# JiehongLin/SAM-6D

Measured on NVIDIA H100. Metric: poses/sec, higher is better.
Workload: dtype bf16

## Files before the change

include/sam6d_b200.h:

```cpp
#ifndef SAM6D_B200_H
#define SAM6D_B200_H

#ifdef __cplusplus
extern "C" {
#endif


int sam6d_fps(const float* xyz, int b, int n, int m, float* temp, int* idx, void* stream);
int sam6d_fps_single_cta(const float* xyz, int b, int n, int m, float* temp, int* idx, void* stream);

int sam6d_gather_points(const float* points, const int* idx, int b, int c, int n, int m, float* out, void* stream);

int sam6d_gather_rows(const float* src, const int* idx, int b, int n, int m, int c, long long src_bstride, float* out,
                      void* stream);
int sam6d_gather_rows_bf16_f32(const void* src, const int* idx, int b, int n, int m, int c, long long src_bstride, float* out,
                               void* stream);

int sam6d_ball_query(const float* new_xyz, const float* xyz, int b, int n, int m, float radius, int nsample, int* idx,
                     int* cnt, void* stream);
int sam6d_ball_query_pair(const float* new_xyz, const float* xyz, int b, int n, int m, float radius_a, int nsample_a,
                          float radius_b, int nsample_b, int* idx_a, int* idx_b, int* cnt_a, int* cnt_b, void* stream);

int sam6d_group_points(const float* points, const int* idx, int b, int c, int n, int np, int ns, float* out, void* stream);

// ... 123 lines not shown
int sam6d_attn_tc_ex(const void* Q, long long q_ld, int q_col0, const void* K, long long k_ld, int k_col0, const void* Vt,
                     long long vt_ld, int B, int H, int Sq, int Sk, int head_dim, float scale, int k_brows, int k_row0, int v_col0,
                     float* lse, void* out, int out_is_bf16, long long out_ld, void* stream);
int sam6d_attn_merge_key(const void* Q, long long q_ld, int q_col0, const void* K, long long k_ld, int k_col0, int k_brows,
                         int key_row, const void* Vt, long long vt_ld, int key_col, const float* lse, int B, int H, int Sq,
                         float scale, void* out, long long out_ld, void* stream);
int sam6d_transpose_tokens_bf16(const void* src, long long ld, int col0, int C, int nB, int L, int N1, void* out, void* stream);
int sam6d_linattn_kv(const float* Kf, long long k_ld, long long k_bs, const float* V, long long v_ld, long long v_bs, int B,
                     int H, int J, float* KV, float* KS, void* stream);
int sam6d_linattn_apply(const float* Qf, long long q_rpb, long long q_bs, long long q_ld, const float* KV, const float* KS,
                        int B, int H, float* X, long long x_bs, long long x_ld, void* stream);
int sam6d_linattn_kv_pack(const float* Kf, long long k_ld, long long k_bs, const float* V, long long v_ld, long long v_bs, int B,
                          int J, void* blob, float* KS, void* stream);
int sam6d_linattn_tc(const void* Q, long long q_ld, long long q_bs, const void* blob, const float* KS,
                     const float* softplus_scale, int B, int rpb, void* X, long long x_ld, long long x_bs, void* stream);

int sam6d_coarse_assign(const float* A, int B, int S, float* W, float* w1, void* stream);
int sam6d_coarse_sample(const float* W, int B, int L, const float* rand, int nr, int* idx, void* stream);
int sam6d_coarse_hypotheses(const int* idx, const float* pts1, const float* pts2, int B, int n, int n1, float* Rt,
                            float* resid, void* stream);
int sam6d_topk_smallest(const float* v, int B, int n, int k, int* out, void* stream);
int sam6d_coarse_select(const float* Rt, const int* top, int B, int n1, int n2, const float* pts1, const float* w1, int n,
                        const float* model, int nm, float* scores, float* R, float* t, void* stream);
int sam6d_coarse_pick_distinct(const float* Rt, const int* top, const float* scores, int B, int n1, int n2, int K, float cos_thr,
                               float d2_min, float* R_out, float* t_out, float* score_out, unsigned char* valid, int* count,
                               void* stream);
int sam6d_coarse_pick_distinct_sym(const float* Rt, const int* top, const float* scores, int B, int n1, int n2, int K, float cos_thr,
                                   float d2_min, const float* symR, const float* symt, int S, const int* sym_range, int max_count,
                                   const float* radius, float* R_out, float* t_out, float* score_out, unsigned char* valid,
                                   int* count, void* stream);
// ... 95 lines not shown
```

sam6d_b200/csrc/linattn_tc.cu:

```cuda
#include "tc.cuh"

namespace {

constexpr int H = 4, D = 64, C = H * D;
constexpr int A_SLAB = 128 * 128;
constexpr int B_SLAB = 64 * 128;
constexpr int BLOB_BYTES = H * B_SLAB;
constexpr int LT_THREADS = 256;
constexpr int LT_SMEM = H * A_SLAB + H * B_SLAB + 128 * H * 4 + 1024;

__global__ void __launch_bounds__(1024) linattn_kv_pack_kernel(const float* __restrict__ Kf, long long k_ld, long long k_bs,
                                                               const float* __restrict__ V, long long v_ld, long long v_bs, int J,
                                                               uint8_t* __restrict__ blob, float* __restrict__ KS) {
  extern __shared__ __align__(16) float sm[];
  float* ks = sm;
  float* vs = ks + J * D;
  const int bh = blockIdx.x, b = bh / H, h = bh - b * H, tid = threadIdx.x;
  for (int e = tid; e < J * D; e += 1024) {
    int j = e / D, c = e - j * D;
    ks[e] = Kf[(size_t)b * k_bs + (size_t)j * k_ld + h * D + c];
    vs[e] = V[(size_t)b * v_bs + (size_t)j * v_ld + h * D + c];
  }
  __syncthreads();
  const int d = tid >> 4, e0 = (tid & 15) * 4;
  float4 acc = make_float4(0.f, 0.f, 0.f, 0.f);
  float ksum = 0.f;
#pragma unroll 4
  for (int j = 0; j < J; ++j) {
    const float kd = ks[j * D + d];
    const float4 v = *reinterpret_cast<const float4*>(vs + j * D + e0);
    ksum += kd;
    acc.x = fmaf(kd, v.x, acc.x); acc.y = fmaf(kd, v.y, acc.y); acc.z = fmaf(kd, v.z, acc.z); acc.w = fmaf(kd, v.w, acc.w);
  }
  uint8_t* slab = blob + (size_t)b * BLOB_BYTES + h * B_SLAB;
  *reinterpret_cast<__nv_bfloat16*>(slab + tc::sw128_offset(e0 + 0, d)) = __float2bfloat16(acc.x);
  *reinterpret_cast<__nv_bfloat16*>(slab + tc::sw128_offset(e0 + 1, d)) = __float2bfloat16(acc.y);
// ... 15 lines not shown
  uint8_t* a_s = smem;
  uint8_t* b_s = smem + H * A_SLAB;
  float* zs = reinterpret_cast<float*>(b_s + H * B_SLAB);
  __shared__ __align__(8) uint64_t blob_bar;

  const int tid = threadIdx.x, warp = tid >> 5, lane = tid & 31;
  const int b = blockIdx.x / a.tiles_per_cloud, tile = blockIdx.x - b * a.tiles_per_cloud;
  if (tid == 0) {
    tc::mbar_init(&blob_bar, 1);
    tc::mbar_fence_init();
    tc::mbar_arrive_expect_tx(&blob_bar, BLOB_BYTES);
    tc::bulk_load_1d(b_s, a.blob + (size_t)b * BLOB_BYTES, BLOB_BYTES, &blob_bar);
  }

  float rs[8], ksv[8];
  {
    const float4 s0 = *reinterpret_cast<const float4*>(a.sp_scale + lane * 8), s1 = *reinterpret_cast<const float4*>(a.sp_scale + lane * 8 + 4);
    rs[0] = 1.f / s0.x; rs[1] = 1.f / s0.y; rs[2] = 1.f / s0.z; rs[3] = 1.f / s0.w;
    rs[4] = 1.f / s1.x; rs[5] = 1.f / s1.y; rs[6] = 1.f / s1.z; rs[7] = 1.f / s1.w;
    const float4 k0 = *reinterpret_cast<const float4*>(a.KS + (size_t)b * C + lane * 8), k1 = *reinterpret_cast<const float4*>(a.KS + (size_t)b * C + lane * 8 + 4);
    ksv[0] = k0.x; ksv[1] = k0.y; ksv[2] = k0.z; ksv[3] = k0.w; ksv[4] = k1.x; ksv[5] = k1.y; ksv[6] = k1.z; ksv[7] = k1.w;
  }
  const int head = lane >> 3, piece = lane & 7;
  const __nv_bfloat16* qbase = a.Q + (size_t)b * a.q_bs + (size_t)tile * 128 * a.q_ld + lane * 8;
  const int rows_left = a.rpb - tile * 128;
#pragma unroll 1
  for (int i0 = warp; i0 < 128; i0 += 32) {
    uint4 raw[4];
#pragma unroll
    for (int u = 0; u < 4; ++u) {
      const int i = i0 + u * 8;
      raw[u] = (i < rows_left) ? *reinterpret_cast<const uint4*>(qbase + (size_t)i * a.q_ld) : make_uint4(0u, 0u, 0u, 0u);
    }
#pragma unroll
    for (int u = 0; u < 4; ++u) {
      const int i = i0 + u * 8;
      const uint32_t w[4] = {raw[u].x, raw[u].y, raw[u].z, raw[u].w};
      float q[8];
      float s1 = 0.f, s3 = 0.f;
#pragma unroll
      for (int e = 0; e < 4; ++e) {
        q[2 * e] = __uint_as_float(w[e] << 16);
        q[2 * e + 1] = __uint_as_float(w[e] & 0xffff0000u);
      }
#pragma unroll
      for (int e = 0; e < 8; ++e) {
        float t = (fmaxf(q[e], 0.f) + 1e-6f) * rs[e];
        s1 = fmaf(t, t, s1);
        t = t * t * t;
        s3 = fmaf(t, t, s3);
        q[e] = t;
      }
      s1 = warp_sum(s1);
      s3 = warp_sum(s3);
      const float n = sqrtf(s1) * rsqrtf(s3);
      float zp = 0.f;
#pragma unroll
      for (int e = 0; e < 8; ++e) { q[e] *= n; zp = fmaf(q[e], ksv[e], zp); }
      zp += __shfl_xor_sync(0xffffffffu, zp, 1);
      zp += __shfl_xor_sync(0xffffffffu, zp, 2);
      zp += __shfl_xor_sync(0xffffffffu, zp, 4);
      const bool valid = i < rows_left;
      if (piece == 0) zs[i * H + head] = valid ? 1.f / (zp + 1e-6f) : 0.f;
      uint4 o = make_uint4(0u, 0u, 0u, 0u);
      if (valid) o = make_uint4(tc::pack_bf16(q[0], q[1]), tc::pack_bf16(q[2], q[3]), tc::pack_bf16(q[4], q[5]), tc::pack_bf16(q[6], q[7]));
      *reinterpret_cast<uint4*>(a_s + head * A_SLAB + i * 128 + ((piece ^ (i & 7)) << 4)) = o;
    }
  }
  tc::fence_proxy_async_smem();
  __syncthreads();

  const int wg = warp >> 2, w = warp & 3;
  tc::mbar_wait(&blob_bar, 0);
  __nv_bfloat16* xb = a.X + (size_t)b * a.x_bs;
#pragma unroll 1
  for (int h = 0; h < H; ++h) {
    float acc[D / 2];
    const uint32_t a_addr = tc::smem_u32(a_s + h * A_SLAB) + wg * (64 * 128), b_addr = tc::smem_u32(b_s + h * B_SLAB);
    tc::wg_fence();
#pragma unroll
// ... 1 lines not shown
    tc::wg_commit();
    tc::wg_wait<0>();
#pragma unroll
    for (int hr = 0; hr < 2; ++hr) {
      const int r = wg * 64 + tc::frag_row(2 * hr, w, lane), row = tile * 128 + r;
      if (row >= a.rpb) continue;
      const float z = zs[r * H + h];
#pragma unroll
      for (int j = 0; j < D / 8; ++j)
        *reinterpret_cast<uint32_t*>(xb + (size_t)row * a.x_ld + h * D + tc::frag_col(4 * j, lane)) =
            tc::pack_bf16(acc[4 * j + 2 * hr] * z, acc[4 * j + 2 * hr + 1] * z);
    }
  }
}

}

S6_API int sam6d_linattn_kv_pack(const float* Kf, long long k_ld, long long k_bs, const float* V, long long v_ld, long long v_bs,
                                 int B, int J, void* blob, float* KS, void* stream) {
  S6_REQUIRE(Kf && V && blob && KS && B >= 0 && J > 0);
  if (B == 0) return 0;
  size_t smem = (size_t)2 * J * D * sizeof(float);
  S6_REQUIRE(smem <= 200 * 1024);
  S6_CHECK(cudaFuncSetAttribute(linattn_kv_pack_kernel, cudaFuncAttributeMaxDynamicSharedMemorySize, (int)smem));
  linattn_kv_pack_kernel<<<B * H, 1024, smem, s6_stream(stream)>>>(Kf, k_ld, k_bs, V, v_ld, v_bs, J, reinterpret_cast<uint8_t*>(blob), KS);
  S6_LAUNCH_CHECK();
  return 0;
}

S6_API int sam6d_linattn_tc(const void* Q, long long q_ld, long long q_bs, const void* blob, const float* KS,
                            const float* softplus_scale, int B, int rpb, void* X, long long x_ld, long long x_bs, void* stream) {
  S6_REQUIRE(Q && blob && KS && softplus_scale && X && B >= 0 && rpb >= 0 && (q_ld % 8) == 0 && (x_ld % 8) == 0 &&
             (q_bs % 8) == 0 && (x_bs % 8) == 0);
  S6_REQUIRE((reinterpret_cast<uintptr_t>(Q) & 15) == 0 && (reinterpret_cast<uintptr_t>(X) & 15) == 0 &&
             (reinterpret_cast<uintptr_t>(blob) & 15) == 0 && (long long)B * rpb < 2000000000LL);
  if (B == 0 || rpb == 0) return 0;
  S6_CHECK(cudaFuncSetAttribute(linattn_tc_kernel, cudaFuncAttributeMaxDynamicSharedMemorySize, LT_SMEM));
  LtArgs a{reinterpret_cast<const __nv_bfloat16*>(Q), q_ld, q_bs, reinterpret_cast<const uint8_t*>(blob), KS, softplus_scale,
           reinterpret_cast<__nv_bfloat16*>(X), x_ld, x_bs, rpb, s6_cdiv(rpb, 128)};
  linattn_tc_kernel<<<B * a.tiles_per_cloud, LT_THREADS, LT_SMEM, s6_stream(stream)>>>(a);
  S6_LAUNCH_CHECK();
  return 0;
// ... 2 lines not shown
```

sam6d_b200/csrc/rowops.cu:

```cuda
#include "common.cuh"

namespace {

struct RowView {
  long long rpb, bstride, ld;
  __device__ __forceinline__ size_t off(long long r) const {
    long long b = r / rpb, i = r - b * rpb;
    return (size_t)(b * bstride + i * ld);
  }
};

constexpr int MAXV_LIMIT = 64;

__device__ __forceinline__ void st_out(float* p, float v) { *p = v; }
__device__ __forceinline__ void st_out(__nv_bfloat16* p, float v) { *p = __float2bfloat16(v); }

__device__ __forceinline__ float ld_in(const float* p) { return *p; }
__device__ __forceinline__ float ld_in(const __nv_bfloat16* p) { return __bfloat162float(*p); }

template <int MAXV, typename OT, typename IT = float>
__global__ void __launch_bounds__(256) layernorm_kernel(const IT* __restrict__ x, RowView xv, OT* __restrict__ y, RowView yv,
                                                        const float* __restrict__ gamma, const float* __restrict__ beta,
                                                        long long rows, int C, float eps) {
  const int lane = threadIdx.x & 31;
// ... 113 lines not shown
  const float n = fmaxf(sqrtf(warp_sum(s)), 1e-12f);
#pragma unroll
  for (int i = 0; i < MAXV; ++i)
    if (i < nv) st_out(yp + lane + 32 * i, v[i] / n);
}

template <int MAXV>
__global__ void __launch_bounds__(256) focus_kernel(const float* __restrict__ x, RowView xv, float* __restrict__ y, RowView yv,
                                                    const float* __restrict__ sp_scale, long long rows, int C) {
  const int lane = threadIdx.x & 31;
  const long long r = (long long)blockIdx.x * 8 + (threadIdx.x >> 5);
  if (r >= rows) return;
  const float* xp = x + xv.off(r);
  float* yp = y + yv.off(r);
  const int nv = C >> 5;
  float v[MAXV];
  float s1 = 0.f, s3 = 0.f;
#pragma unroll
  for (int i = 0; i < MAXV; ++i)
    if (i < nv) {
      int c = lane + 32 * i;
      float q = (fmaxf(xp[c], 0.f) + 1e-6f) / sp_scale[c];
      s1 += q * q;
      q = q * q * q;
      s3 += q * q;
      v[i] = q;
    }
  const float n1 = sqrtf(warp_sum(s1)), n3 = sqrtf(warp_sum(s3));
#pragma unroll
  for (int i = 0; i < MAXV; ++i)
    if (i < nv) yp[lane + 32 * i] = (v[i] / n3) * n1;
}

__global__ void rigid_warp_kernel(const float* __restrict__ p, const float* __restrict__ R, const float* __restrict__ t, int n,
                                  long long total, float* __restrict__ out) {
  long long i = (long long)blockIdx.x * blockDim.x + threadIdx.x;
  if (i >= total) return;
  int b = (int)(i / n);
  const float* Rb = R + (size_t)b * 9;
  const float* tb = t + (size_t)b * 3;
  float x = p[i * 3 + 0] - tb[0], y = p[i * 3 + 1] - tb[1], z = p[i * 3 + 2] - tb[2];
  out[i * 3 + 0] = x * Rb[0] + y * Rb[3] + z * Rb[6];
  out[i * 3 + 1] = x * Rb[1] + y * Rb[4] + z * Rb[7];
// ... 165 lines not shown
```

sam6d_b200/csrc/tail_tc.cu:

```cuda
#include "tc.cuh"

namespace {

constexpr int BM = 128, C = 256, HID = 512, BK = 64;
constexpr int T_SLAB = BM * 128;
constexpr int T_BYTES = 4 * T_SLAB;
constexpr int W_STAGE = 256 * 128;
constexpr int W_STAGES = 3;
constexpr int W_PER_TILE = 20;
constexpr int CONSUMERS = 256, THREADS = CONSUMERS + 128;
constexpr int SMEM = 2 * T_BYTES + W_STAGES * W_STAGE + 1024;

struct TailArgs {
  const float* bo; const float* g1; const float* b1;
  const float* be; const float* bs; const float* g2; const float* b2;
  int M;
  float eps;
};

__device__ __forceinline__ uint32_t* tile_pair(uint8_t* tile, int r, int col) {
  return reinterpret_cast<uint32_t*>(tile + (col >> 6) * T_SLAB + r * 128 + ((((col & 63) >> 3) ^ (r & 7)) << 4) + (col & 7) * 2);
}
__device__ __forceinline__ float2 unpack2(uint32_t w) { return make_float2(__uint_as_float(w << 16), __uint_as_float(w & 0xffff0000u)); }

__global__ void __launch_bounds__(THREADS, 1) tail_tc_kernel(const __grid_constant__ CUtensorMap tmHid, const __grid_constant__ CUtensorMap tmX,
                                                const __grid_constant__ CUtensorMap tmWo, const __grid_constant__ CUtensorMap tmWe,
                                                const __grid_constant__ CUtensorMap tmWs, TailArgs a, __nv_bfloat16* __restrict__ out,
                                                long long ld_out) {
  extern __shared__ __align__(1024) uint8_t smem_raw[];
  uint8_t* smem = reinterpret_cast<uint8_t*>((reinterpret_cast<uintptr_t>(smem_raw) + 1023) & ~(uintptr_t)1023);
  uint8_t* a_buf = smem;
  uint8_t* x_buf = smem + T_BYTES;
  uint8_t* w_ring = smem + 2 * T_BYTES;
  __shared__ __align__(8) uint64_t in_full, in_empty, w_full[W_STAGES], w_empty[W_STAGES];

  const int tid = threadIdx.x, warp = tid >> 5, lane = tid & 31;
  const int ntiles = (a.M + BM - 1) / BM;

  if (tid == 0) {
    tc::mbar_init(&in_full, 1); tc::mbar_init(&in_empty, CONSUMERS / 32);
    for (int s = 0; s < W_STAGES; ++s) { tc::mbar_init(&w_full[s], 1); tc::mbar_init(&w_empty[s], CONSUMERS / 32); }
    tc::mbar_fence_init();
    tc::tma_prefetch_desc(&tmHid); tc::tma_prefetch_desc(&tmX); tc::tma_prefetch_desc(&tmWo);
    tc::tma_prefetch_desc(&tmWe); tc::tma_prefetch_desc(&tmWs);
  }
  s6_pdl_trigger();
  if (tid < CONSUMERS) {
    for (int i = tid; i < 512; i += CONSUMERS) {
      const float* p = i < 64 ? a.bo + i * 4 : i < 128 ? a.g1 + (i - 64) * 4 : i < 192 ? a.b1 + (i - 128) * 4 : i < 320 ? a.be + (i - 192) * 4
                     : i < 384 ? a.bs + (i - 320) * 4 : i < 448 ? a.g2 + (i - 384) * 4 : a.b2 + (i - 448) * 4;
      asm volatile("prefetch.global.L1 [%0];" ::"l"(p));
    }
  }
  __syncthreads();
  s6_pdl_wait();

  if (warp >= CONSUMERS / 32) {
    tc::producer_regs();
    if (tid == CONSUMERS) {
      long long gw = 0;
      int it = 0;
      for (int tile = blockIdx.x; tile < ntiles; tile += gridDim.x, ++it) {
        const int m0 = tile * BM;
        auto load_w = [&](int j) {
          const int s = (int)(gw % W_STAGES);
          tc::mbar_wait(&w_empty[s], (uint32_t)(((gw / W_STAGES) & 1) ^ 1));
          tc::mbar_arrive_expect_tx(&w_full[s], W_STAGE);
          uint8_t* dst = w_ring + s * W_STAGE;
          if (j < 4) tc::tma_load_2d(&tmWo, &w_full[s], dst, j * BK, 0);
          else if (j < 12) tc::tma_load_2d(&tmWe, &w_full[s], dst, ((j - 4) & 3) * BK, ((j - 4) >> 2) * 256);
          else tc::tma_load_2d(&tmWs, &w_full[s], dst, (j - 12) * BK, 0);
          ++gw;
        };
        int j = 0;
        for (; j < W_STAGES; ++j) load_w(j);
        tc::mbar_wait(&in_empty, (uint32_t)((it & 1) ^ 1));
        tc::mbar_arrive_expect_tx(&in_full, 2 * T_BYTES);
#pragma unroll
        for (int kb = 0; kb < 4; ++kb) {
          tc::tma_load_2d(&tmHid, &in_full, a_buf + kb * T_SLAB, kb * BK, m0);
          tc::tma_load_2d(&tmX, &in_full, x_buf + kb * T_SLAB, kb * BK, m0);
        }
        for (; j < W_PER_TILE; ++j) load_w(j);
      }
    }
    return;
  }
  tc::consumer_regs();
  const int wg = warp >> 2, w = warp & 3;
  const uint32_t a_addr = tc::smem_u32(a_buf) + wg * (64 * 128), x_addr = tc::smem_u32(x_buf) + wg * (64 * 128), w_addr0 = tc::smem_u32(w_ring);
  long long gw = 0;
  float acc[C / 2];
  auto gemm = [&](uint32_t op_addr, uint32_t op_addr2, int nkb) {
    int prev = -1;
    for (int kb = 0; kb < nkb; ++kb, ++gw) {
      const int s = (int)(gw % W_STAGES);
      tc::mbar_wait(&w_full[s], (uint32_t)((gw / W_STAGES) & 1));
      const uint32_t op = (kb < 4 ? op_addr : op_addr2) + (kb & 3) * T_SLAB;
      tc::wg_fence();
#pragma unroll
      for (int k = 0; k < 4; ++k)
        tc::wgmma_bf16<C>(acc, tc::wg_desc(op + k * 32), tc::wg_desc(w_addr0 + s * W_STAGE + k * 32), (kb | k) ? 1u : 0u);
      tc::wg_commit();
      if (prev >= 0) {
// ... 31 lines not shown
  };
  auto relu_store = [&](const float* __restrict__ bias, uint8_t* dst) {
#pragma unroll
    for (int e = 0; e < C / 2; e += 2) {
      const int col = tc::frag_col(e, lane), r = wg * 64 + tc::frag_row(e, w, lane);
      const float2 bb = __ldg(reinterpret_cast<const float2*>(bias + col));
      *tile_pair(dst, r, col) = tc::pack_bf16(fmaxf(acc[e] + bb.x, 0.f), fmaxf(acc[e + 1] + bb.y, 0.f));
    }
  };
  auto publish = [&]() {
    tc::fence_proxy_async_smem();
    tc::named_bar(1 + wg, 128);
  };
  int it = 0;
  for (int tile = blockIdx.x; tile < ntiles; tile += gridDim.x, ++it) {
    tc::mbar_wait(&in_full, (uint32_t)(it & 1));
    gemm(a_addr, a_addr, 4);
    layernorm(a.bo, a.g1, a.b1, [&](int e, int hr, int col) {
      return unpack2(*tile_pair(x_buf, wg * 64 + tc::frag_row(e, w, lane), col));
    });
#pragma unroll
    for (int e = 0; e < C / 2; e += 2) {
      const int r = wg * 64 + tc::frag_row(e, w, lane), col = tc::frag_col(e, lane), row = tile * BM + r;
      const uint32_t y2 = tc::pack_bf16(acc[e], acc[e + 1]);
      *tile_pair(a_buf, r, col) = y2;
      if (row < a.M) *reinterpret_cast<uint32_t*>(out + (size_t)row * ld_out + col) = y2;
    }
    publish();
    gemm(a_addr, a_addr, 4);
    relu_store(a.be, x_buf);
    gemm(a_addr, a_addr, 4);
    tc::named_bar(1 + wg, 128);
    relu_store(a.be + 256, a_buf);
    publish();
    gemm(x_addr, a_addr, 8);
    if (lane == 0) tc::mbar_arrive(&in_empty);
    layernorm(a.bs, a.g2, a.b2, [&](int e, int, int col) {
      const int row = tile * BM + wg * 64 + tc::frag_row(e, w, lane);
      return row < a.M ? unpack2(*reinterpret_cast<const uint32_t*>(out + (size_t)row * ld_out + col)) : make_float2(0.f, 0.f);
    });
#pragma unroll
    for (int e = 0; e < C / 2; e += 2) {
      const int row = tile * BM + wg * 64 + tc::frag_row(e, w, lane);
      if (row < a.M) *reinterpret_cast<uint32_t*>(out + (size_t)row * ld_out + tc::frag_col(e, lane)) = tc::pack_bf16(acc[e], acc[e + 1]);
    }
  }
}

}

S6_API int sam6d_transformer_tail_bf16(const void* hid, long long ld_hid, const void* x, long long ld_x, const void* Wo, const float* bo,
                                       const float* g1, const float* b1, const void* We, const float* be, const void* Ws, const float* bs,
                                       const float* g2, const float* b2, void* out, long long ld_out, int M, float eps, void* stream) {
  S6_REQUIRE(hid && x && Wo && bo && g1 && b1 && We && be && Ws && bs && g2 && b2 && out && M >= 0);
  S6_REQUIRE((ld_hid % 8) == 0 && (ld_x % 8) == 0 && (ld_out % 8) == 0 && ld_hid >= C && ld_x >= C && ld_out >= C);
  S6_REQUIRE(((reinterpret_cast<uintptr_t>(hid) | reinterpret_cast<uintptr_t>(x) | reinterpret_cast<uintptr_t>(out) | reinterpret_cast<uintptr_t>(Wo) |
               reinterpret_cast<uintptr_t>(We) | reinterpret_cast<uintptr_t>(Ws) | reinterpret_cast<uintptr_t>(bo) | reinterpret_cast<uintptr_t>(be) |
               reinterpret_cast<uintptr_t>(bs) | reinterpret_cast<uintptr_t>(g1) | reinterpret_cast<uintptr_t>(b1) | reinterpret_cast<uintptr_t>(g2) |
               reinterpret_cast<uintptr_t>(b2)) & 15) == 0);
  if (M == 0) return 0;
  CUtensorMap tmHid, tmX, tmWo, tmWe, tmWs;
  int rc;
  if ((rc = tc::make_map_2d(&tmHid, hid, M, C, ld_hid, 64, BM))) return rc;
  if ((rc = tc::make_map_2d(&tmX, x, M, C, ld_x, 64, BM))) return rc;
  if ((rc = tc::make_map_2d(&tmWo, Wo, C, C, C, 64, 256))) return rc;
  if ((rc = tc::make_map_2d(&tmWe, We, HID, C, C, 64, 256))) return rc;
  if ((rc = tc::make_map_2d(&tmWs, Ws, C, HID, HID, 64, 256))) return rc;
  int grid;
  S6_CHECK(s6_persistent_grid(s6_cdiv(M, BM), 1, &grid));
  TailArgs a{bo, g1, b1, be, bs, g2, b2, M, eps};
  S6_CHECK(cudaFuncSetAttribute(tail_tc_kernel, cudaFuncAttributeMaxDynamicSharedMemorySize, SMEM));
  S6_CHECK(s6_launch_pdl(tail_tc_kernel, dim3(grid), dim3(THREADS), SMEM, s6_stream(stream), tmHid, tmX, tmWo, tmWe, tmWs, a,
                         reinterpret_cast<__nv_bfloat16*>(out), ld_out));
  S6_LAUNCH_CHECK();
  return 0;
}
```

sam6d_b200/ops.py:

```python
from typing import Optional, Tuple

import numpy as np
import torch

from . import _lib

Tensor = torch.Tensor


def _check(t: Tensor, dtype, name: str, ndim: Optional[int] = None):
    if not isinstance(t, torch.Tensor):
        raise RuntimeError(f"{name} must be a torch.Tensor")
    if not t.is_cuda:
        raise RuntimeError(f"{name} must be a CUDA tensor (CPU not supported)")
    if t.dtype != dtype:
        raise RuntimeError(f"{name} must be {dtype}, got {t.dtype}")
    if not t.is_contiguous():
        raise RuntimeError(f"{name} must be contiguous")
    if ndim is not None and t.dim() != ndim:
        raise RuntimeError(f"{name} must have {ndim} dims, got {t.dim()}")


def _rows(t: Tensor) -> Tuple[int, int, int]:
    if t.dim() not in (2, 3) or t.stride(-1) != 1:
# ... 524 lines not shown


def linattn_apply(q: Tensor, KV: Tensor, KS: Tensor, out: Tensor):
    _, x_bs, x_ld = _rows(out)
    _lib.call("sam6d_linattn_apply", q, *_rows(q), KV, KS, q.shape[0], KV.shape[1], out, x_bs, x_ld)


def linattn_kv_pack(k: Tensor, v: Tensor) -> Tuple[Tensor, Tensor]:
    B, J, _ = k.shape
    _, k_bs, k_ld = _rows(k)
    _, v_bs, v_ld = _rows(v)
    blob = torch.empty(B, 4 * 64 * 64, dtype=torch.bfloat16, device=k.device)
    KS = torch.empty(B, 4, 64, dtype=torch.float32, device=k.device)
    _lib.call("sam6d_linattn_kv_pack", k, k_ld, k_bs, v, v_ld, v_bs, B, J, blob, KS)
    return blob, KS


def linattn_tc(q: Tensor, blob: Tensor, KS: Tensor, sp_scale: Tensor, out: Tensor):
    B, rpb, _ = q.shape
    _, q_bs, q_ld = _rows(q)
    _, x_bs, x_ld = _rows(out)
    _lib.call("sam6d_linattn_tc", q, q_ld, q_bs, blob, KS, sp_scale, B, rpb, out, x_ld, x_bs)


def coarse_assign(A: Tensor) -> Tuple[Tensor, Tensor]:
    _check(A, torch.float32, "atten", 3)
    B, S, _ = A.shape
    n = S - 1
    W = torch.empty(B, n * n, dtype=torch.float32, device=A.device)
    w1 = torch.empty(B, n, dtype=torch.float32, device=A.device)
# ... 471 lines not shown
```

sam6d_b200/pem.py:

```python
import math
from types import SimpleNamespace
from typing import Dict, Optional

import torch
import torch.nn as nn

from . import ops
from .layers import _W, _f32, _gemm, _Packed, _param_key, PRECISIONS

NUM_HEADS = 4

RPE_TC = True
PADDED_BIAS = True
GEO_LUT_INV_H = 8.0
GEO_LUT_D_MAX = 32.0


def _cfg(cfg, **defaults):
    if isinstance(cfg, dict):
        cfg = SimpleNamespace(**cfg)
    for k, v in defaults.items():
        if not hasattr(cfg, k):
            setattr(cfg, k, v)
    return cfg
# ... 488 lines not shown
    def _pack(self):
        la = self.dense_layer.attention.attention
        return dict(
            wq=_W(la.proj_q.weight), bq=_f32(la.proj_q.bias),
            wkv=_W(torch.cat([_f32(la.proj_k.weight), _f32(la.proj_v.weight)], dim=0)),
            bkv=torch.cat([_f32(la.proj_k.bias), _f32(la.proj_v.bias)], dim=0).contiguous(),
            sp_scale=torch.nn.functional.softplus(_f32(la.scale)).reshape(-1).contiguous(), tail=_pack_tail(self.dense_layer))

    def _sample_feats(self, dense_feats, idx_ext):
        if dense_feats.dtype == torch.bfloat16:
            return ops.gather_rows_bf16(dense_feats, idx_ext)
        return ops.gather_rows(dense_feats, idx_ext)

    def _dense_layer_bf16(self, dense, sparse, w):
        B, N1, C = dense.shape
        N, J = N1 - 1, sparse.shape[1] - 1
        dev = dense.device
        bf = torch.bfloat16
        x2d = dense.view(B * N1, C)
        q = ops.gemm_tma(x2d, w["wq"].bf16, w["bq"], out_dtype=bf)
        kv = torch.empty(B * J, 2 * C, dtype=torch.float32, device=dev)
        ops.gemm_tc(sparse[:, 1:, :], w["wkv"].bf16, w["bkv"], out=kv.view(B, J, 2 * C))
        ops.focus_rows(kv[:, :C], w["sp_scale"], out=kv[:, :C])
        kv3 = kv.view(B, J, 2 * C)
        blob, KS = ops.linattn_kv_pack(kv3[..., :C], kv3[..., C:])
        x_att = torch.empty(B * N1, C, dtype=bf, device=dev)
        ops.linattn_tc(q.view(B, N1, C)[:, 1:, :], blob, KS, w["sp_scale"], x_att.view(B, N1, C)[:, 1:, :])
        x_att.view(B, N1, C)[:, 0, :] = 0
        out = _tail_bf16(x2d, x_att, w["tail"]).view(B, N1, C)
        out[:, 0, :] = sparse[:, 0, :].to(bf)
        return out

    def _dense_layer(self, dense, sparse, w):
        B, N1, C = dense.shape
        N, J = N1 - 1, sparse.shape[1] - 1
        dev = dense.device
        x = dense[:, 1:, :]
        q = torch.empty(B * N, C, dtype=torch.float32, device=dev)
        prec = self.precision
        _gemm(prec, x, w["wq"], w["bq"], out=q.view(B, N, C))
        kv = torch.empty(B * J, 2 * C, dtype=torch.float32, device=dev)
        _gemm(prec, sparse[:, 1:, :], w["wkv"], w["bkv"], out=kv.view(B, J, 2 * C))
        ops.focus_rows(q, w["sp_scale"], out=q)
        ops.focus_rows(kv[:, :C], w["sp_scale"], out=kv[:, :C])
        KV = torch.empty(B, NUM_HEADS, 64, 64, dtype=torch.float32, device=dev)
        KS = torch.empty(B, NUM_HEADS, 64, dtype=torch.float32, device=dev)
# ... 269 lines not shown
```

Measured before the change: 2635.

## Fuse Q projection and linear attention into the persistent tail kernel

```diff
diff --git a/include/sam6d_b200.h b/include/sam6d_b200.h
--- a/include/sam6d_b200.h
+++ b/include/sam6d_b200.h
@@ -161,6 +161,12 @@
                           int J, void* blob, float* KS, void* stream);
 int sam6d_linattn_tc(const void* Q, long long q_ld, long long q_bs, const void* blob, const float* KS,
                      const float* softplus_scale, int B, int rpb, void* X, long long x_ld, long long x_bs, void* stream);
+int sam6d_linattn_kv_focus_pack(const float* K, long long k_ld, long long k_bs, const float* V, long long v_ld, long long v_bs,
+                                const float* softplus_scale, int B, int J, void* blob, float* KS, void* stream);
+int sam6d_linattn_tail_bf16(const void* x, long long ld_x, int B, int N1, const void* Wq, const float* bq, const void* blob,
+                            const float* KS, const float* softplus_scale, const void* bg, long long bg_bs, const void* Wo,
+                            const float* bo, const float* g1, const float* b1, const void* We, const float* be, const void* Ws,
+                            const float* bs, const float* g2, const float* b2, void* out, long long ld_out, float eps, void* stream);
 
 int sam6d_coarse_assign(const float* A, int B, int S, float* W, float* w1, void* stream);
 int sam6d_coarse_sample(const float* W, int B, int L, const float* rand, int nr, int* idx, void* stream);
diff --git a/sam6d_b200/csrc/linattn.cuh b/sam6d_b200/csrc/linattn.cuh
--- /dev/null
+++ b/sam6d_b200/csrc/linattn.cuh
@@ -0,0 +1,64 @@
+#pragma once
+#include "tc.cuh"
+
+namespace linattn {
+
+template <int MAXV>
+__device__ __forceinline__ void focus_f32_row(const float* __restrict__ xp, const float* __restrict__ sp_scale, int nv, int lane,
+                                              float (&v)[MAXV], float& n1, float& n3) {
+  float s1 = 0.f, s3 = 0.f;
+#pragma unroll
+  for (int i = 0; i < MAXV; ++i)
+    if (i < nv) {
+      int c = lane + 32 * i;
+      float q = (fmaxf(xp[c], 0.f) + 1e-6f) / sp_scale[c];
+      s1 += q * q;
+      q = q * q * q;
+      s3 += q * q;
+      v[i] = q;
+    }
+  n1 = sqrtf(warp_sum(s1));
+  n3 = sqrtf(warp_sum(s3));
+}
+
+__device__ __forceinline__ uint4 focus_bf16_row(uint4 raw, const float (&rs)[8], const float (&ksv)[8], bool valid, float& zinv) {
+  const uint32_t w[4] = {raw.x, raw.y, raw.z, raw.w};
+  float q[8];
+  float s1 = 0.f, s3 = 0.f;
+#pragma unroll
+  for (int e = 0; e < 4; ++e) {
+    q[2 * e] = __uint_as_float(w[e] << 16);
+    q[2 * e + 1] = __uint_as_float(w[e] & 0xffff0000u);
+  }
+#pragma unroll
+  for (int e = 0; e < 8; ++e) {
+    float t = (fmaxf(q[e], 0.f) + 1e-6f) * rs[e];
+    s1 = fmaf(t, t, s1);
+    t = t * t * t;
+    s3 = fmaf(t, t, s3);
+    q[e] = t;
+  }
+  s1 = warp_sum(s1);
+  s3 = warp_sum(s3);
+  const float n = sqrtf(s1) * rsqrtf(s3);
+  float zp = 0.f;
+#pragma unroll
+  for (int e = 0; e < 8; ++e) { q[e] *= n; zp = fmaf(q[e], ksv[e], zp); }
+  zp += __shfl_xor_sync(0xffffffffu, zp, 1);
+  zp += __shfl_xor_sync(0xffffffffu, zp, 2);
+  zp += __shfl_xor_sync(0xffffffffu, zp, 4);
+  zinv = valid ? 1.f / (zp + 1e-6f) : 0.f;
+  if (!valid) return make_uint4(0u, 0u, 0u, 0u);
+  return make_uint4(tc::pack_bf16(q[0], q[1]), tc::pack_bf16(q[2], q[3]), tc::pack_bf16(q[4], q[5]), tc::pack_bf16(q[6], q[7]));
+}
+
+__device__ __forceinline__ void focus_bf16_consts(const float* __restrict__ sp_scale, const float* __restrict__ KS, int b, int lane,
+                                                  float (&rs)[8], float (&ksv)[8]) {
+  const float4 s0 = *reinterpret_cast<const float4*>(sp_scale + lane * 8), s1 = *reinterpret_cast<const float4*>(sp_scale + lane * 8 + 4);
+  rs[0] = 1.f / s0.x; rs[1] = 1.f / s0.y; rs[2] = 1.f / s0.z; rs[3] = 1.f / s0.w;
+  rs[4] = 1.f / s1.x; rs[5] = 1.f / s1.y; rs[6] = 1.f / s1.z; rs[7] = 1.f / s1.w;
+  const float4 k0 = *reinterpret_cast<const float4*>(KS + (size_t)b * 256 + lane * 8), k1 = *reinterpret_cast<const float4*>(KS + (size_t)b * 256 + lane * 8 + 4);
+  ksv[0] = k0.x; ksv[1] = k0.y; ksv[2] = k0.z; ksv[3] = k0.w; ksv[4] = k1.x; ksv[5] = k1.y; ksv[6] = k1.z; ksv[7] = k1.w;
+}
+
+}
diff --git a/sam6d_b200/csrc/linattn_tc.cu b/sam6d_b200/csrc/linattn_tc.cu
--- a/sam6d_b200/csrc/linattn_tc.cu
+++ b/sam6d_b200/csrc/linattn_tc.cu
@@ -1,4 +1,4 @@
-#include "tc.cuh"
+#include "linattn.cuh"
 
 namespace {
 
@@ -9,17 +9,37 @@
 constexpr int LT_THREADS = 256;
 constexpr int LT_SMEM = H * A_SLAB + H * B_SLAB + 128 * H * 4 + 1024;
 
-__global__ void __launch_bounds__(1024) linattn_kv_pack_kernel(const float* __restrict__ Kf, long long k_ld, long long k_bs,
+template <bool FOCUS>
+__global__ void __launch_bounds__(1024, 1) linattn_kv_pack_kernel(const float* __restrict__ Kf, long long k_ld, long long k_bs,
                                                                const float* __restrict__ V, long long v_ld, long long v_bs, int J,
-                                                               uint8_t* __restrict__ blob, float* __restrict__ KS) {
+                                                               const float* __restrict__ sp_scale, uint8_t* __restrict__ blob,
+                                                               float* __restrict__ KS) {
   extern __shared__ __align__(16) float sm[];
   float* ks = sm;
   float* vs = ks + J * D;
   const int bh = blockIdx.x, b = bh / H, h = bh - b * H, tid = threadIdx.x;
-  for (int e = tid; e < J * D; e += 1024) {
-    int j = e / D, c = e - j * D;
-    ks[e] = Kf[(size_t)b * k_bs + (size_t)j * k_ld + h * D + c];
-    vs[e] = V[(size_t)b * v_bs + (size_t)j * v_ld + h * D + c];
+  if constexpr (FOCUS) {
+    const int warp = tid >> 5, lane = tid & 31;
+    for (int j = warp; j < J; j += 32) {
+      float v[8], n1, n3;
+      linattn::focus_f32_row(Kf + (size_t)b * k_bs + (size_t)j * k_ld, sp_scale, 8, lane, v, n1, n3);
+      float lo = v[0], hi = v[1];
+#pragma unroll
+      for (int i = 2; i < 8; i += 2)
+        if ((i >> 1) == h) { lo = v[i]; hi = v[i + 1]; }
+      ks[j * D + lane] = (lo / n3) * n1;
+      ks[j * D + lane + 32] = (hi / n3) * n1;
+    }
+    for (int e = tid; e < J * D; e += 1024) {
+      int j = e / D, c = e - j * D;
+      vs[e] = V[(size_t)b * v_bs + (size_t)j * v_ld + h * D + c];
+    }
+  } else {
+    for (int e = tid; e < J * D; e += 1024) {
+      int j = e / D, c = e - j * D;
+      ks[e] = Kf[(size_t)b * k_bs + (size_t)j * k_ld + h * D + c];
+      vs[e] = V[(size_t)b * v_bs + (size_t)j * v_ld + h * D + c];
+    }
   }
   __syncthreads();
   const int d = tid >> 4, e0 = (tid & 15) * 4;
@@ -65,13 +85,7 @@
   }
 
   float rs[8], ksv[8];
-  {
-    const float4 s0 = *reinterpret_cast<const float4*>(a.sp_scale + lane * 8), s1 = *reinterpret_cast<const float4*>(a.sp_scale + lane * 8 + 4);
-    rs[0] = 1.f / s0.x; rs[1] = 1.f / s0.y; rs[2] = 1.f / s0.z; rs[3] = 1.f / s0.w;
-    rs[4] = 1.f / s1.x; rs[5] = 1.f / s1.y; rs[6] = 1.f / s1.z; rs[7] = 1.f / s1.w;
-    const float4 k0 = *reinterpret_cast<const float4*>(a.KS + (size_t)b * C + lane * 8), k1 = *reinterpret_cast<const float4*>(a.KS + (size_t)b * C + lane * 8 + 4);
-    ksv[0] = k0.x; ksv[1] = k0.y; ksv[2] = k0.z; ksv[3] = k0.w; ksv[4] = k1.x; ksv[5] = k1.y; ksv[6] = k1.z; ksv[7] = k1.w;
-  }
+  linattn::focus_bf16_consts(a.sp_scale, a.KS, b, lane, rs, ksv);
   const int head = lane >> 3, piece = lane & 7;
   const __nv_bfloat16* qbase = a.Q + (size_t)b * a.q_bs + (size_t)tile * 128 * a.q_ld + lane * 8;
   const int rows_left = a.rpb - tile * 128;
@@ -86,35 +100,9 @@
 #pragma unroll
     for (int u = 0; u < 4; ++u) {
       const int i = i0 + u * 8;
-      const uint32_t w[4] = {raw[u].x, raw[u].y, raw[u].z, raw[u].w};
-      float q[8];
-      float s1 = 0.f, s3 = 0.f;
-#pragma unroll
-      for (int e = 0; e < 4; ++e) {
-        q[2 * e] = __uint_as_float(w[e] << 16);
-        q[2 * e + 1] = __uint_as_float(w[e] & 0xffff0000u);
-      }
-#pragma unroll
-      for (int e = 0; e < 8; ++e) {
-        float t = (fmaxf(q[e], 0.f) + 1e-6f) * rs[e];
-        s1 = fmaf(t, t, s1);
-        t = t * t * t;
-        s3 = fmaf(t, t, s3);
-        q[e] = t;
-      }
-      s1 = warp_sum(s1);
-      s3 = warp_sum(s3);
-      const float n = sqrtf(s1) * rsqrtf(s3);
-      float zp = 0.f;
-#pragma unroll
-      for (int e = 0; e < 8; ++e) { q[e] *= n; zp = fmaf(q[e], ksv[e], zp); }
-      zp += __shfl_xor_sync(0xffffffffu, zp, 1);
-      zp += __shfl_xor_sync(0xffffffffu, zp, 2);
-      zp += __shfl_xor_sync(0xffffffffu, zp, 4);
-      const bool valid = i < rows_left;
-      if (piece == 0) zs[i * H + head] = valid ? 1.f / (zp + 1e-6f) : 0.f;
-      uint4 o = make_uint4(0u, 0u, 0u, 0u);
-      if (valid) o = make_uint4(tc::pack_bf16(q[0], q[1]), tc::pack_bf16(q[2], q[3]), tc::pack_bf16(q[4], q[5]), tc::pack_bf16(q[6], q[7]));
+      float zinv;
+      const uint4 o = linattn::focus_bf16_row(raw[u], rs, ksv, i < rows_left, zinv);
+      if (piece == 0) zs[i * H + head] = zinv;
       *reinterpret_cast<uint4*>(a_s + head * A_SLAB + i * 128 + ((piece ^ (i & 7)) << 4)) = o;
     }
   }
@@ -146,18 +134,30 @@
   }
 }
 
+int launch_kv_pack(const float* Kf, long long k_ld, long long k_bs, const float* V, long long v_ld, long long v_bs, int B, int J,
+                   const float* sp_scale, void* blob, float* KS, void* stream) {
+  S6_REQUIRE(Kf && V && blob && KS && B >= 0 && J > 0);
+  if (B == 0) return 0;
+  size_t smem = (size_t)2 * J * D * sizeof(float);
+  S6_REQUIRE(smem <= 200 * 1024);
+  auto kern = sp_scale ? linattn_kv_pack_kernel<true> : linattn_kv_pack_kernel<false>;
+  S6_CHECK(cudaFuncSetAttribute(kern, cudaFuncAttributeMaxDynamicSharedMemorySize, (int)smem));
+  kern<<<B * H, 1024, smem, s6_stream(stream)>>>(Kf, k_ld, k_bs, V, v_ld, v_bs, J, sp_scale, reinterpret_cast<uint8_t*>(blob), KS);
+  S6_LAUNCH_CHECK();
+  return 0;
+}
+
 }
 
 S6_API int sam6d_linattn_kv_pack(const float* Kf, long long k_ld, long long k_bs, const float* V, long long v_ld, long long v_bs,
                                  int B, int J, void* blob, float* KS, void* stream) {
-  S6_REQUIRE(Kf && V && blob && KS && B >= 0 && J > 0);
-  if (B == 0) return 0;
-  size_t smem = (size_t)2 * J * D * sizeof(float);
-  S6_REQUIRE(smem <= 200 * 1024);
-  S6_CHECK(cudaFuncSetAttribute(linattn_kv_pack_kernel, cudaFuncAttributeMaxDynamicSharedMemorySize, (int)smem));
-  linattn_kv_pack_kernel<<<B * H, 1024, smem, s6_stream(stream)>>>(Kf, k_ld, k_bs, V, v_ld, v_bs, J, reinterpret_cast<uint8_t*>(blob), KS);
-  S6_LAUNCH_CHECK();
-  return 0;
+  return launch_kv_pack(Kf, k_ld, k_bs, V, v_ld, v_bs, B, J, nullptr, blob, KS, stream);
+}
+
+S6_API int sam6d_linattn_kv_focus_pack(const float* K, long long k_ld, long long k_bs, const float* V, long long v_ld, long long v_bs,
+                                       const float* softplus_scale, int B, int J, void* blob, float* KS, void* stream) {
+  S6_REQUIRE(softplus_scale != nullptr);
+  return launch_kv_pack(K, k_ld, k_bs, V, v_ld, v_bs, B, J, softplus_scale, blob, KS, stream);
 }
 
 S6_API int sam6d_linattn_tc(const void* Q, long long q_ld, long long q_bs, const void* blob, const float* KS,
diff --git a/sam6d_b200/csrc/rowops.cu b/sam6d_b200/csrc/rowops.cu
--- a/sam6d_b200/csrc/rowops.cu
+++ b/sam6d_b200/csrc/rowops.cu
@@ -1,4 +1,5 @@
 #include "common.cuh"
+#include "linattn.cuh"
 
 namespace {
 
@@ -151,19 +152,8 @@
   const float* xp = x + xv.off(r);
   float* yp = y + yv.off(r);
   const int nv = C >> 5;
-  float v[MAXV];
-  float s1 = 0.f, s3 = 0.f;
-#pragma unroll
-  for (int i = 0; i < MAXV; ++i)
-    if (i < nv) {
-      int c = lane + 32 * i;
-      float q = (fmaxf(xp[c], 0.f) + 1e-6f) / sp_scale[c];
-      s1 += q * q;
-      q = q * q * q;
-      s3 += q * q;
-      v[i] = q;
-    }
-  const float n1 = sqrtf(warp_sum(s1)), n3 = sqrtf(warp_sum(s3));
+  float v[MAXV], n1, n3;
+  linattn::focus_f32_row(xp, sp_scale, nv, lane, v, n1, n3);
 #pragma unroll
   for (int i = 0; i < MAXV; ++i)
     if (i < nv) yp[lane + 32 * i] = (v[i] / n3) * n1;
diff --git a/sam6d_b200/csrc/tail_tc.cu b/sam6d_b200/csrc/tail_tc.cu
--- a/sam6d_b200/csrc/tail_tc.cu
+++ b/sam6d_b200/csrc/tail_tc.cu
@@ -1,4 +1,4 @@
-#include "tc.cuh"
+#include "linattn.cuh"
 
 namespace {
 
@@ -8,14 +8,23 @@
 constexpr int W_STAGE = 256 * 128;
 constexpr int W_STAGES = 3;
 constexpr int W_PER_TILE = 20;
+constexpr int LA_STAGES = 5;
 constexpr int CONSUMERS = 256, THREADS = CONSUMERS + 128;
-constexpr int SMEM = 2 * T_BYTES + W_STAGES * W_STAGE + 1024;
+constexpr int ZS_BYTES = BM * 4 * 4, BAR_BYTES = 128;
+constexpr int SMEM = 2 * T_BYTES + W_STAGES * W_STAGE + ZS_BYTES + BAR_BYTES + 896;
+static_assert(SMEM <= 227 * 1024, "exceeds the shared memory of one CTA");
+static_assert(W_STAGE == 4 * 64 * 128, "one ring stage holds the four [64][64] KV_h^T slabs of a cloud");
 
 struct TailArgs {
   const float* bo; const float* g1; const float* b1;
   const float* be; const float* bs; const float* g2; const float* b2;
-  int M;
+  int rpc;
+  int clouds;
+  long long cloud_rows;
+  int row0;
   float eps;
+  const float* bq; const float* sp_scale; const uint8_t* blob; const float* KS;
+  const __nv_bfloat16* bg; long long bg_bs;
 };
 
 __device__ __forceinline__ uint32_t* tile_pair(uint8_t* tile, int r, int col) {
@@ -23,6 +32,7 @@
 }
 __device__ __forceinline__ float2 unpack2(uint32_t w) { return make_float2(__uint_as_float(w << 16), __uint_as_float(w & 0xffff0000u)); }
 
+template <bool LA>
 __global__ void __launch_bounds__(THREADS, 1) tail_tc_kernel(const __grid_constant__ CUtensorMap tmHid, const __grid_constant__ CUtensorMap tmX,
                                                 const __grid_constant__ CUtensorMap tmWo, const __grid_constant__ CUtensorMap tmWe,
                                                 const __grid_constant__ CUtensorMap tmWs, TailArgs a, __nv_bfloat16* __restrict__ out,
@@ -32,12 +42,17 @@
   uint8_t* a_buf = smem;
   uint8_t* x_buf = smem + T_BYTES;
   uint8_t* w_ring = smem + 2 * T_BYTES;
-  __shared__ __align__(8) uint64_t in_full, in_empty, w_full[W_STAGES], w_empty[W_STAGES];
+  float* zs = reinterpret_cast<float*>(w_ring + W_STAGES * W_STAGE);
+  uint64_t* bars = reinterpret_cast<uint64_t*>(zs + BM * 4);
+  uint64_t &in_full = bars[0], &in_empty = bars[1], *w_full = bars + 2, *w_empty = bars + 2 + W_STAGES;
+  constexpr int W_TILE = LA ? LA_STAGES + W_PER_TILE : W_PER_TILE;
+  constexpr int W_TAIL = LA ? LA_STAGES : 0;
 
   const int tid = threadIdx.x, warp = tid >> 5, lane = tid & 31;
-  const int ntiles = (a.M + BM - 1) / BM;
+  const int tpc = (a.rpc + BM - 1) / BM, ntiles = tpc * a.clouds;
 
   if (tid == 0) {
+    if (LA && reinterpret_cast<uint8_t*>(bars) + BAR_BYTES > smem_raw + SMEM) __trap();
     tc::mbar_init(&in_full, 1); tc::mbar_init(&in_empty, CONSUMERS / 32);
     for (int s = 0; s < W_STAGES; ++s) { tc::mbar_init(&w_full[s], 1); tc::mbar_init(&w_empty[s], CONSUMERS / 32); }
     tc::mbar_fence_init();
@@ -61,13 +76,15 @@
       long long gw = 0;
       int it = 0;
       for (int tile = blockIdx.x; tile < ntiles; tile += gridDim.x, ++it) {
-        const int m0 = tile * BM;
+        const int cloud = tile / tpc, m0 = (int)(cloud * a.cloud_rows) + a.row0 + (tile - cloud * tpc) * BM;
         auto load_w = [&](int j) {
           const int s = (int)(gw % W_STAGES);
           tc::mbar_wait(&w_empty[s], (uint32_t)(((gw / W_STAGES) & 1) ^ 1));
           tc::mbar_arrive_expect_tx(&w_full[s], W_STAGE);
           uint8_t* dst = w_ring + s * W_STAGE;
-          if (j < 4) tc::tma_load_2d(&tmWo, &w_full[s], dst, j * BK, 0);
+          if (LA && j < 4) tc::tma_load_2d(&tmHid, &w_full[s], dst, j * BK, 0);
+          else if (LA && j == 4) tc::bulk_load_1d(dst, a.blob + (size_t)cloud * W_STAGE, W_STAGE, &w_full[s]);
+          else if ((j -= W_TAIL) < 4) tc::tma_load_2d(&tmWo, &w_full[s], dst, j * BK, 0);
           else if (j < 12) tc::tma_load_2d(&tmWe, &w_full[s], dst, ((j - 4) & 3) * BK, ((j - 4) >> 2) * 256);
           else tc::tma_load_2d(&tmWs, &w_full[s], dst, (j - 12) * BK, 0);
           ++gw;
@@ -75,19 +92,25 @@
         int j = 0;
         for (; j < W_STAGES; ++j) load_w(j);
         tc::mbar_wait(&in_empty, (uint32_t)((it & 1) ^ 1));
-        tc::mbar_arrive_expect_tx(&in_full, 2 * T_BYTES);
+        tc::mbar_arrive_expect_tx(&in_full, (LA ? 1 : 2) * T_BYTES);
 #pragma unroll
         for (int kb = 0; kb < 4; ++kb) {
-          tc::tma_load_2d(&tmHid, &in_full, a_buf + kb * T_SLAB, kb * BK, m0);
+          if (!LA) tc::tma_load_2d(&tmHid, &in_full, a_buf + kb * T_SLAB, kb * BK, m0);
           tc::tma_load_2d(&tmX, &in_full, x_buf + kb * T_SLAB, kb * BK, m0);
         }
-        for (; j < W_PER_TILE; ++j) load_w(j);
+        for (; j < W_TILE; ++j) load_w(j);
       }
     }
     return;
   }
   tc::consumer_regs();
   const int wg = warp >> 2, w = warp & 3;
+  if constexpr (LA) {
+    for (int i = blockIdx.x * CONSUMERS + tid; i < a.clouds * (C / 8); i += gridDim.x * CONSUMERS) {
+      const int b = i / (C / 8), c = (i - b * (C / 8)) * 8;
+      *reinterpret_cast<uint4*>(out + (size_t)b * a.cloud_rows * ld_out + c) = *reinterpret_cast<const uint4*>(a.bg + (size_t)b * a.bg_bs + c);
+    }
+  }
   const uint32_t a_addr = tc::smem_u32(a_buf) + wg * (64 * 128), x_addr = tc::smem_u32(x_buf) + wg * (64 * 128), w_addr0 = tc::smem_u32(w_ring);
   long long gw = 0;
   float acc[C / 2];
@@ -149,17 +172,67 @@
   };
   int it = 0;
   for (int tile = blockIdx.x; tile < ntiles; tile += gridDim.x, ++it) {
+    const int cloud = tile / tpc, t0 = (tile - cloud * tpc) * BM;
+    __nv_bfloat16* const out_t = out + ((size_t)cloud * a.cloud_rows + a.row0 + t0) * ld_out;
+    const int rows = a.rpc - t0;
     tc::mbar_wait(&in_full, (uint32_t)(it & 1));
+    if constexpr (LA) {
+      gemm(x_addr, x_addr, 4);
+#pragma unroll
+      for (int e = 0; e < C / 2; e += 2) {
+        const int r = wg * 64 + tc::frag_row(e, w, lane), col = tc::frag_col(e, lane);
+        const float2 bb = __ldg(reinterpret_cast<const float2*>(a.bq + col));
+        *tile_pair(a_buf, r, col) = tc::pack_bf16(fmaf(acc[e], 1.f, bb.x), fmaf(acc[e + 1], 1.f, bb.y));
+      }
+      tc::named_bar(1 + wg, 128);
+      float rs[8], ksv[8];
+      linattn::focus_bf16_consts(a.sp_scale, a.KS, cloud, lane, rs, ksv);
+      const int head = lane >> 3, piece = lane & 7;
+#pragma unroll 4
+      for (int i = 0; i < 16; ++i) {
+        const int r = wg * 64 + w + 4 * i;
+        uint4* p = reinterpret_cast<uint4*>(a_buf + head * T_SLAB + r * 128 + ((piece ^ (r & 7)) << 4));
+        float zinv;
+        const uint4 o = linattn::focus_bf16_row(*p, rs, ksv, r < rows, zinv);
+        if (piece == 0) zs[r * 4 + head] = zinv;
+        *p = o;
+      }
+      tc::fence_proxy_async_smem();
+      tc::named_bar(1 + wg, 128);
+      const int s = (int)(gw % W_STAGES);
+      tc::mbar_wait(&w_full[s], (uint32_t)((gw / W_STAGES) & 1));
+#pragma unroll 1
+      for (int h = 0; h < 4; ++h) {
+        float xa[32];
+        const uint32_t qa = a_addr + h * T_SLAB, kva = w_addr0 + s * W_STAGE + h * (64 * 128);
+        tc::wg_fence();
+#pragma unroll
+        for (int k = 0; k < 4; ++k) tc::wgmma_bf16<64>(xa, tc::wg_desc(qa + k * 32), tc::wg_desc(kva + k * 32), k ? 1u : 0u);
+        tc::wg_commit();
+        tc::wg_wait<0>();
+#pragma unroll
+        for (int hr = 0; hr < 2; ++hr) {
+          const int r = wg * 64 + tc::frag_row(2 * hr, w, lane);
+          const float z = zs[r * 4 + h];
+#pragma unroll
+          for (int j = 0; j < 8; ++j)
+            *tile_pair(a_buf, r, h * 64 + tc::frag_col(4 * j, lane)) = tc::pack_bf16(xa[4 * j + 2 * hr] * z, xa[4 * j + 2 * hr + 1] * z);
+        }
+      }
+      if (lane == 0) tc::mbar_arrive(&w_empty[s]);
+      ++gw;
+      publish();
+    }
     gemm(a_addr, a_addr, 4);
     layernorm(a.bo, a.g1, a.b1, [&](int e, int hr, int col) {
       return unpack2(*tile_pair(x_buf, wg * 64 + tc::frag_row(e, w, lane), col));
     });
 #pragma unroll
     for (int e = 0; e < C / 2; e += 2) {
-      const int r = wg * 64 + tc::frag_row(e, w, lane), col = tc::frag_col(e, lane), row = tile * BM + r;
+      const int r = wg * 64 + tc::frag_row(e, w, lane), col = tc::frag_col(e, lane);
       const uint32_t y2 = tc::pack_bf16(acc[e], acc[e + 1]);
       *tile_pair(a_buf, r, col) = y2;
-      if (row < a.M) *reinterpret_cast<uint32_t*>(out + (size_t)row * ld_out + col) = y2;
+      if (r < rows) *reinterpret_cast<uint32_t*>(out_t + (size_t)r * ld_out + col) = y2;
     }
     publish();
     gemm(a_addr, a_addr, 4);
@@ -171,15 +244,38 @@
     gemm(x_addr, a_addr, 8);
     if (lane == 0) tc::mbar_arrive(&in_empty);
     layernorm(a.bs, a.g2, a.b2, [&](int e, int, int col) {
-      const int row = tile * BM + wg * 64 + tc::frag_row(e, w, lane);
-      return row < a.M ? unpack2(*reinterpret_cast<const uint32_t*>(out + (size_t)row * ld_out + col)) : make_float2(0.f, 0.f);
+      const int r = wg * 64 + tc::frag_row(e, w, lane);
+      return r < rows ? unpack2(*reinterpret_cast<const uint32_t*>(out_t + (size_t)r * ld_out + col)) : make_float2(0.f, 0.f);
     });
 #pragma unroll
     for (int e = 0; e < C / 2; e += 2) {
-      const int row = tile * BM + wg * 64 + tc::frag_row(e, w, lane);
-      if (row < a.M) *reinterpret_cast<uint32_t*>(out + (size_t)row * ld_out + tc::frag_col(e, lane)) = tc::pack_bf16(acc[e], acc[e + 1]);
-    }
-  }
+      const int r = wg * 64 + tc::frag_row(e, w, lane);
+      if (r < rows) *reinterpret_cast<uint32_t*>(out_t + (size_t)r * ld_out + tc::frag_col(e, lane)) = tc::pack_bf16(acc[e], acc[e + 1]);
+    }
+  }
+}
+
+template <bool LA>
+int launch_tail(const CUtensorMap& tmHid, const CUtensorMap& tmX, const void* Wo, const void* We, const void* Ws, const TailArgs& a,
+                void* out, long long ld_out, void* stream) {
+  CUtensorMap tmWo, tmWe, tmWs;
+  int rc;
+  if ((rc = tc::make_map_2d(&tmWo, Wo, C, C, C, 64, 256))) return rc;
+  if ((rc = tc::make_map_2d(&tmWe, We, HID, C, C, 64, 256))) return rc;
+  if ((rc = tc::make_map_2d(&tmWs, Ws, C, HID, HID, 64, 256))) return rc;
+  int grid;
+  S6_CHECK(s6_persistent_grid((long long)s6_cdiv(a.rpc, BM) * a.clouds, 1, &grid));
+  S6_CHECK(cudaFuncSetAttribute(tail_tc_kernel<LA>, cudaFuncAttributeMaxDynamicSharedMemorySize, SMEM));
+  S6_CHECK(s6_launch_pdl(tail_tc_kernel<LA>, dim3(grid), dim3(THREADS), SMEM, s6_stream(stream), tmHid, tmX, tmWo, tmWe, tmWs, a,
+                         reinterpret_cast<__nv_bfloat16*>(out), ld_out));
+  S6_LAUNCH_CHECK();
+  return 0;
+}
+
+bool aligned16(std::initializer_list<const void*> ps) {
+  uintptr_t u = 0;
+  for (const void* p : ps) u |= reinterpret_cast<uintptr_t>(p);
+  return (u & 15) == 0;
 }
 
 }
@@ -189,24 +285,31 @@
                                        const float* g2, const float* b2, void* out, long long ld_out, int M, float eps, void* stream) {
   S6_REQUIRE(hid && x && Wo && bo && g1 && b1 && We && be && Ws && bs && g2 && b2 && out && M >= 0);
   S6_REQUIRE((ld_hid % 8) == 0 && (ld_x % 8) == 0 && (ld_out % 8) == 0 && ld_hid >= C && ld_x >= C && ld_out >= C);
-  S6_REQUIRE(((reinterpret_cast<uintptr_t>(hid) | reinterpret_cast<uintptr_t>(x) | reinterpret_cast<uintptr_t>(out) | reinterpret_cast<uintptr_t>(Wo) |
-               reinterpret_cast<uintptr_t>(We) | reinterpret_cast<uintptr_t>(Ws) | reinterpret_cast<uintptr_t>(bo) | reinterpret_cast<uintptr_t>(be) |
-               reinterpret_cast<uintptr_t>(bs) | reinterpret_cast<uintptr_t>(g1) | reinterpret_cast<uintptr_t>(b1) | reinterpret_cast<uintptr_t>(g2) |
-               reinterpret_cast<uintptr_t>(b2)) & 15) == 0);
+  S6_REQUIRE(aligned16({hid, x, out, Wo, We, Ws, bo, be, bs, g1, b1, g2, b2}));
   if (M == 0) return 0;
-  CUtensorMap tmHid, tmX, tmWo, tmWe, tmWs;
+  CUtensorMap tmHid, tmX;
   int rc;
   if ((rc = tc::make_map_2d(&tmHid, hid, M, C, ld_hid, 64, BM))) return rc;
   if ((rc = tc::make_map_2d(&tmX, x, M, C, ld_x, 64, BM))) return rc;
-  if ((rc = tc::make_map_2d(&tmWo, Wo, C, C, C, 64, 256))) return rc;
-  if ((rc = tc::make_map_2d(&tmWe, We, HID, C, C, 64, 256))) return rc;
-  if ((rc = tc::make_map_2d(&tmWs, Ws, C, HID, HID, 64, 256))) return rc;
-  int grid;
-  S6_CHECK(s6_persistent_grid(s6_cdiv(M, BM), 1, &grid));
-  TailArgs a{bo, g1, b1, be, bs, g2, b2, M, eps};
-  S6_CHECK(cudaFuncSetAttribute(tail_tc_kernel, cudaFuncAttributeMaxDynamicSharedMemorySize, SMEM));
-  S6_CHECK(s6_launch_pdl(tail_tc_kernel, dim3(grid), dim3(THREADS), SMEM, s6_stream(stream), tmHid, tmX, tmWo, tmWe, tmWs, a,
-                         reinterpret_cast<__nv_bfloat16*>(out), ld_out));
-  S6_LAUNCH_CHECK();
-  return 0;
-}
+  TailArgs a{bo, g1, b1, be, bs, g2, b2, M, 1, 0, 0, eps, nullptr, nullptr, nullptr, nullptr, nullptr, 0};
+  return launch_tail<false>(tmHid, tmX, Wo, We, Ws, a, out, ld_out, stream);
+}
+
+S6_API int sam6d_linattn_tail_bf16(const void* x, long long ld_x, int B, int N1, const void* Wq, const float* bq, const void* blob,
+                                   const float* KS, const float* softplus_scale, const void* bg, long long bg_bs, const void* Wo,
+                                   const float* bo, const float* g1, const float* b1, const void* We, const float* be, const void* Ws,
+                                   const float* bs, const float* g2, const float* b2, void* out, long long ld_out, float eps,
+                                   void* stream) {
+  S6_REQUIRE(x && Wq && bq && blob && KS && softplus_scale && bg && Wo && bo && g1 && b1 && We && be && Ws && bs && g2 && b2 && out);
+  S6_REQUIRE(B >= 0 && N1 >= 1 && (long long)B * N1 < 2000000000LL && (ld_x % 8) == 0 && (ld_out % 8) == 0 && (bg_bs % 8) == 0 &&
+             ld_x >= C && ld_out >= C);
+  S6_REQUIRE(aligned16({x, out, Wq, bq, blob, KS, softplus_scale, bg, Wo, We, Ws, bo, be, bs, g1, b1, g2, b2}));
+  if (B == 0) return 0;
+  CUtensorMap tmWq, tmX;
+  int rc;
+  if ((rc = tc::make_map_2d(&tmWq, Wq, C, C, C, 64, 256))) return rc;
+  if ((rc = tc::make_map_2d(&tmX, x, (long long)B * N1, C, ld_x, 64, BM))) return rc;
+  TailArgs a{bo, g1, b1, be, bs, g2, b2, N1 - 1, B, N1, 1, eps, bq, softplus_scale, reinterpret_cast<const uint8_t*>(blob), KS,
+             reinterpret_cast<const __nv_bfloat16*>(bg), bg_bs};
+  return launch_tail<true>(tmWq, tmX, Wo, We, Ws, a, out, ld_out, stream);
+}
diff --git a/sam6d_b200/ops.py b/sam6d_b200/ops.py
--- a/sam6d_b200/ops.py
+++ b/sam6d_b200/ops.py
@@ -562,6 +562,31 @@
     KS = torch.empty(B, 4, 64, dtype=torch.float32, device=k.device)
     _lib.call("sam6d_linattn_kv_pack", k, k_ld, k_bs, v, v_ld, v_bs, B, J, blob, KS)
     return blob, KS
+
+
+def linattn_kv_focus_pack(k: Tensor, v: Tensor, sp_scale: Tensor) -> Tuple[Tensor, Tensor]:
+    B, J, _ = k.shape
+    _, k_bs, k_ld = _rows(k)
+    _, v_bs, v_ld = _rows(v)
+    blob = torch.empty(B, 4 * 64 * 64, dtype=torch.bfloat16, device=k.device)
+    KS = torch.empty(B, 4, 64, dtype=torch.float32, device=k.device)
+    _lib.call("sam6d_linattn_kv_focus_pack", k, k_ld, k_bs, v, v_ld, v_bs, sp_scale, B, J, blob, KS)
+    return blob, KS
+
+
+def linattn_tail_bf16(x: Tensor, wq: Tensor, bq: Tensor, blob: Tensor, KS: Tensor, sp_scale: Tensor, bg: Tensor, wo: Tensor,
+                      bo: Tensor, g1: Tensor, b1: Tensor, we: Tensor, be: Tensor, ws: Tensor, bs: Tensor, g2: Tensor, b2: Tensor,
+                      eps: float = 1e-5) -> Tensor:
+    _check(x, torch.bfloat16, "x", 3)
+    B, N1, C = x.shape
+    if C != 256 or bg.dtype != torch.bfloat16 or not bg.is_cuda or bg.shape != (B, C) or bg.stride(1) != 1:
+        raise RuntimeError("linattn_tail_bf16: x (B,N1,256) contiguous, bg (B,256) rows")
+    for w in (wq, wo, we, ws):
+        _check(w, torch.bfloat16, "weight", 2)
+    out = torch.empty_like(x)
+    _lib.call("sam6d_linattn_tail_bf16", x, C, B, N1, wq, bq, blob, KS, sp_scale, bg, bg.stride(0), wo, bo, g1, b1, we, be, ws, bs,
+              g2, b2, out, C, eps)
+    return out
 
 
 def linattn_tc(q: Tensor, blob: Tensor, KS: Tensor, sp_scale: Tensor, out: Tensor):
diff --git a/sam6d_b200/pem.py b/sam6d_b200/pem.py
--- a/sam6d_b200/pem.py
+++ b/sam6d_b200/pem.py
@@ -526,22 +526,13 @@
 
     def _dense_layer_bf16(self, dense, sparse, w):
         B, N1, C = dense.shape
-        N, J = N1 - 1, sparse.shape[1] - 1
-        dev = dense.device
-        bf = torch.bfloat16
-        x2d = dense.view(B * N1, C)
-        q = ops.gemm_tma(x2d, w["wq"].bf16, w["bq"], out_dtype=bf)
-        kv = torch.empty(B * J, 2 * C, dtype=torch.float32, device=dev)
-        ops.gemm_tc(sparse[:, 1:, :], w["wkv"].bf16, w["bkv"], out=kv.view(B, J, 2 * C))
-        ops.focus_rows(kv[:, :C], w["sp_scale"], out=kv[:, :C])
-        kv3 = kv.view(B, J, 2 * C)
-        blob, KS = ops.linattn_kv_pack(kv3[..., :C], kv3[..., C:])
-        x_att = torch.empty(B * N1, C, dtype=bf, device=dev)
-        ops.linattn_tc(q.view(B, N1, C)[:, 1:, :], blob, KS, w["sp_scale"], x_att.view(B, N1, C)[:, 1:, :])
-        x_att.view(B, N1, C)[:, 0, :] = 0
-        out = _tail_bf16(x2d, x_att, w["tail"]).view(B, N1, C)
-        out[:, 0, :] = sparse[:, 0, :].to(bf)
-        return out
+        J = sparse.shape[1] - 1
+        kv = torch.empty(B, J, 2 * C, dtype=torch.float32, device=dense.device)
+        ops.gemm_tc(sparse[:, 1:, :], w["wkv"].bf16, w["bkv"], out=kv)
+        blob, KS = ops.linattn_kv_focus_pack(kv[..., :C], kv[..., C:], w["sp_scale"])
+        t = w["tail"]
+        return ops.linattn_tail_bf16(dense, w["wq"].bf16, w["bq"], blob, KS, w["sp_scale"], sparse[:, 0, :], t["wo"].bf16, t["bo"],
+                                     t["g1"], t["b1"], t["we"].bf16, t["be"], t["ws"].bf16, t["bs"], t["g2"], t["b2"])
 
     def _dense_layer(self, dense, sparse, w):
         B, N1, C = dense.shape
```

Result: faster. 2704, median of 6 (+2.6%).
